# nikhil-lalgudi/distributed-llm-alignment

Hardware: AMD Instinct MI355X
Metric: preference-samples/sec (whole node), Llama-3-8B DPO at 1/2/4/8 MI355X (higher is better)
Workload: dtype bf16; 1 GPU; model=llama3-8b, global_batch=16, seq_len=1024, parallelism=dp1, micro_batch_pairs=4, grad_accum=4, ref_model=frozen, co-resident, backend=single-process, gemm_selection=tunableop:off

## Files before the change

distributed_llm_alignment_amd/csrc/attention.hip:

```cpp
#include <cstdlib>
#include <stdexcept>
#include <type_traits>
#include "common.h"

#include <cstring>
#include "attn_params.h"

namespace dla {

typedef __attribute__((address_space(3))) s16x4 lds_s16x4;

template <int D>
constexpr int attn_dp() { return (D + 31) / 32 * 32; }

template <int W>
__device__ __forceinline__ int swz(int row, int ch) {
  constexpr int NCH = W / 8;
  constexpr int MASK = (NCH & (NCH - 1)) == 0 ? NCH - 1 : 3;
  const int f = (((row & 3) << 2) | ((row >> 2) & 3)) & MASK;
  return row * W + ((ch ^ f) << 3);
}

__device__ __forceinline__ int ds_swz(int row) { return (row >> 1) & 7; }
__device__ __forceinline__ int ds_off(int row, int c4) { return row * 32 + ((c4 ^ ds_swz(row)) << 2); }
// ... 872 lines not shown
      const int t = static_cast<int>(row % T);
      const int64_t bh = row / T;
      const int hh = static_cast<int>(bh % H), b = static_cast<int>(bh / H);
      a[k] = load_bf16x8(o + b * o_sb + t * o_st + hh * o_sh + c);
      g[k] = load_bf16x8(dout + b * do_sb + t * do_st + hh * do_sh + c);
    }
  }
#pragma unroll
  for (int k = 0; k < kDeltaRows; ++k) {
    float acc = 0.f;
#pragma unroll
    for (int j = 0; j < 8; ++j) acc += bf2f(a[k][j]) * bf2f(g[k][j]);
    for (int off = 1; off < lpr; off <<= 1) acc += __shfl_xor(acc, off, 64);
    if (row0 + k < nrows && (lane % lpr) == 0) delta[row0 + k] = acc;
  }
}

template <bool CAUSAL>
__device__ __forceinline__ void bwd_q_range(int k0, int Tq, int causal_off, int window, int& qt0,
                                            int& qend) {
  int qlo = 0, qhi = Tq;
  if (CAUSAL) {
    qlo = max(0, k0 - causal_off);
    if (window > 0) qhi = min(qhi, k0 + kAttnBwdKeys - 1 - causal_off + window);
  }
  qt0 = (qlo / kAttnBwdQRows) * kAttnBwdQRows;
  qend = max(qhi, qt0);
}

template <int D, bool CAUSAL>
// ... 1114 lines not shown
    case 128: fwd_dispatch<128>(p, causal, st); break;
    default: throw std::invalid_argument("attn_fwd: head_dim must be 64, 80 or 128");
  }
}

void launch_attn_bwd_delta(const bf16_t* o, const bf16_t* dout, int64_t o_sb, int64_t o_st,
                           int64_t o_sh, int64_t do_sb, int64_t do_st, int64_t do_sh, int B,
                           int H, int T, int D, float* delta, hipStream_t st) {
  const int64_t rows = static_cast<int64_t>(B) * H * T;
  if (rows == 0) return;
  const int64_t rows_per_block = 4 * (64 / (D <= 64 ? 8 : 16));
  const unsigned nb = static_cast<unsigned>((rows + rows_per_block - 1) / rows_per_block);
  attn_bwd_delta_kernel<<<nb, 256, 0, st>>>(o, dout, o_sb, o_st, o_sh, do_sb, do_st, do_sh, B, H, T, D, delta);
}

static int attn_bwd_waves() {
  const char* e = std::getenv("DLA_ATTN_BWD_WAVES");
  return (e && std::atoi(e) == 4) ? 4 : 8;
}

bool attn_dq_slab_bf16() {
  const char* e = std::getenv("DLA_ATTN_DQ_BF16");
  return attn_bwd_waves() == 8 && !(e && std::atoi(e) == 0);
}

bool attn_dkv_part_bf16() {
  const char* e = std::getenv("DLA_ATTN_DKV_BF16");
  return attn_bwd_waves() == 8 && !(e && std::atoi(e) == 0);
}

// ... 72 lines not shown
```

distributed_llm_alignment_amd/csrc/bindings.cpp:

```cpp
#include <ATen/ATen.h>
#include <ATen/hip/impl/HIPGuardImplMasqueradingAsCUDA.h>
#include <ATen/hip/impl/HIPStreamMasqueradingAsCUDA.h>
#include <torch/library.h>

#include <hip/hip_runtime_api.h>

#include <algorithm>
#include <cstdint>
#include <cstdlib>
#include <tuple>

#include "attn_params.h"
#include "bind_util.h"

namespace dla {

void launch_norm_fwd(const bf16_t*, const bf16_t*, bf16_t*, const bf16_t*, const bf16_t*, bf16_t*,
                     float*, float*, int, int, float, bool, hipStream_t);
void launch_norm_bwd(const bf16_t*, const bf16_t*, const bf16_t*, const float*, const float*,
                     const bf16_t*, bf16_t*, float*, float*, bf16_t*, bf16_t*, int, int, bool,
                     hipStream_t);
int norm_bwd_grid(int rows);
int norm_wgrad_scratch_rows();
void launch_swiglu_fwd(const bf16_t*, bf16_t*, int64_t, int, hipStream_t);
// ... 49 lines not shown
void launch_attn_fwd(const AttnParams&, int, bool, hipStream_t);
int attn_fwd_set_switch(const char* name, int value);
void launch_attn_bwd_delta(const bf16_t*, const bf16_t*, int64_t, int64_t, int64_t, int64_t,
                           int64_t, int64_t, int, int, int, int, float*, hipStream_t);
void launch_attn_bwd(const AttnBwdParams&, int, bool, hipStream_t);
bool attn_dkv_part_bf16();
bool attn_dq_slab_bf16();
void launch_attn_dq_reduce(const float*, int, int, int, int, int, int, bool, int, int,
                           const int*, const int*, int, bf16_t*, int64_t, int64_t, int64_t,
                           const float*, const float*, const int*, int, hipStream_t, const bf16_t*);
void launch_attn_dkv_reduce(const float*, const float*, int, int, int, int, int, float, bf16_t*,
                            int64_t, int64_t, int64_t, bf16_t*, int64_t, int64_t, int64_t,
                            const float*, const float*, const int*, int, hipStream_t, const bf16_t*,
                            const bf16_t*);
void launch_transpose_bf16(const bf16_t*, int64_t, int64_t, int64_t, bf16_t*, int64_t, hipStream_t);

std::tuple<at::Tensor, at::Tensor, at::Tensor, at::Tensor> norm_fwd(
    const at::Tensor& x, const c10::optional<at::Tensor>& res, const at::Tensor& w,
    const c10::optional<at::Tensor>& b, double eps, bool rms) {
  check_bf16(x, "x");
  check_bf16(w, "w");
  TORCH_CHECK(x.is_contiguous(), "x must be contiguous");
  const int64_t H = x.size(-1);
  TORCH_CHECK(H % 8 == 0 && H <= 8192, "norm_fwd: hidden size must be a multiple of 8 and <= 8192");
  TORCH_CHECK(w.numel() == H && w.is_contiguous(), "w shape");
  const int64_t rows = x.numel() / H;
  TORCH_CHECK(rows < (1ll << 31), "too many rows");
  c10::hip::HIPGuardMasqueradingAsCUDA g(x.device());
  auto y = at::empty_like(x);
  at::Tensor so;
// ... 351 lines not shown

static int attn_bwd_hsplit(int64_t nkb, int64_t Hkv, int64_t B, int64_t group, bool causal, int cus) {
  const int64_t base = nkb * Hkv * B;
  const int64_t target = causal ? 2 * static_cast<int64_t>(cus) : cus;
  int hs = 1;
  while (base * hs < target && group % (2 * hs) == 0) hs *= 2;
  return hs;
}

void attn_bwd(const at::Tensor& dout, const at::Tensor& q, const at::Tensor& k,
              const at::Tensor& v, const at::Tensor& o, const at::Tensor& lse2, at::Tensor& dq,
              at::Tensor& dk, at::Tensor& dv, double scale, bool causal, int64_t causal_off,
              int64_t window, const c10::optional<at::Tensor>& kv_start,
              const c10::optional<at::Tensor>& kv_end, const c10::optional<at::Tensor>& segs,
              const c10::optional<at::Tensor>& rope_cos, const c10::optional<at::Tensor>& rope_sin,
              const c10::optional<at::Tensor>& rope_pos, bool rope_inputs) {
  check_bthd(dout, "dout");
  check_bthd(q, "q");
  check_bthd(k, "k");
  check_bthd(v, "v");
  check_bthd(o, "o");
  check_bthd(dq, "dq");
  check_bthd(dk, "dk");
  check_bthd(dv, "dv");
  check_f32(lse2, "lse2");
  const int64_t B = q.size(0), Tq = q.size(1), Hq = q.size(2), D = q.size(3);
  const int64_t Tk = k.size(1), Hkv = k.size(2);
  TORCH_CHECK(D == 64 || D == 80 || D == 128, "head_dim must be 64, 80 or 128");
  TORCH_CHECK(dout.sizes() == q.sizes() && o.sizes() == q.sizes() && dq.sizes() == q.sizes(),
              "dout/o/dq shape");
  TORCH_CHECK(dk.sizes() == k.sizes() && dv.sizes() == v.sizes(), "dk/dv shape");
  TORCH_CHECK(lse2.is_contiguous() && lse2.numel() == B * Hq * Tq, "lse2 shape");
  TORCH_CHECK(Hkv > 0 && Hq % Hkv == 0, "GQA ratio");
  check_kv_range(kv_start, B, "kv_start");
  check_kv_range(kv_end, B, "kv_end");
  c10::hip::HIPGuardMasqueradingAsCUDA g(q.device());
  auto st = cur_stream(q);
  auto fopt = q.options().dtype(at::kFloat);
  auto delta = at::empty({B, Hq, Tq}, fopt);
  launch_attn_bwd_delta(cbp(o), cbp(dout), o.stride(0), o.stride(1), o.stride(2),
                        dout.stride(0), dout.stride(1), dout.stride(2), B, Hq, Tq, D,
                        delta.data_ptr<float>(), st);
  const int64_t nkb = (Tk + kAttnBwdKeys - 1) / kAttnBwdKeys;
  const int64_t slab_rows = (Tq + kAttnBwdQRows - 1) / kAttnBwdQRows * kAttnBwdQRows;
  const bool slab16 = attn_dq_slab_bf16();
  auto slab = at::empty({std::max<int64_t>(nkb, 1), B, slab_rows, Hq, D}, slab16 ? q.options() : fopt);
  const int hs = attn_bwd_hsplit(nkb, Hkv, B, Hq / Hkv, causal, device_cus(q.get_device()));
  at::Tensor dkp, dvp;
  const bool part16 = hs > 1 && attn_dkv_part_bf16();
  if (hs > 1) {
    dkp = at::empty({hs, B, Tk, Hkv, D}, part16 ? q.options() : fopt);
    dvp = at::empty({hs, B, Tk, Hkv, D}, part16 ? q.options() : fopt);
  }
  AttnBwdParams p{};
  p.q = cbp(q); p.k = cbp(k); p.v = cbp(v); p.dout = cbp(dout);
  p.lse2 = lse2.data_ptr<float>(); p.delta = delta.data_ptr<float>();
  p.dq_slab = slab16 ? nullptr : slab.data_ptr<float>();
// ... 27 lines not shown
  launch_attn_bwd(p, static_cast<int>(D), causal, st);
  launch_attn_dq_reduce(p.dq_slab, static_cast<int>(nkb), static_cast<int>(B), static_cast<int>(Tq),
                        p.slab_rows, static_cast<int>(Hq), static_cast<int>(D), causal, p.causal_off, p.window,
                        p.kv_start, p.kv_end, static_cast<int>(Tk), bp(dq), dq.stride(0),
                        dq.stride(1), dq.stride(2), p.rope_cos, p.rope_sin, p.rope_pos, p.rope_rot, st,
                        p.dq_slab16);
  if (hs > 1) {
    launch_attn_dkv_reduce(p.dk_part, p.dv_part, hs, static_cast<int>(B), static_cast<int>(Tk),
                           static_cast<int>(Hkv), static_cast<int>(D), p.scale, bp(dk),
                           dk.stride(0), dk.stride(1), dk.stride(2), bp(dv), dv.stride(0),
                           dv.stride(1), dv.stride(2), p.rope_cos, p.rope_sin, p.rope_pos, p.rope_rot, st,
                           p.dk_part16, p.dv_part16);
  }
}

void transpose_bf16(const at::Tensor& in, at::Tensor& out) {
  check_bf16(in, "in");
  check_bf16(out, "out");
  TORCH_CHECK(in.dim() == 2 && out.dim() == 2 && in.stride(1) == 1 && out.stride(1) == 1 &&
                  out.size(0) == in.size(1) && out.size(1) == in.size(0),
              "transpose_bf16: in [R, C], out [C, R], unit column stride");
  TORCH_CHECK(in.stride(0) % 8 == 0 && out.stride(0) % 8 == 0, "16-byte aligned rows");
  check_aligned16(in, "in");
  check_aligned16(out, "out");
  same_device(in, out);
  c10::hip::HIPGuardMasqueradingAsCUDA g(in.device());
  launch_transpose_bf16(cbp(in), in.size(0), in.size(1), in.stride(0), bp(out), out.stride(0),
                        cur_stream(in));
}

// ... 434 lines not shown

}

TORCH_LIBRARY(dla, m) {
  m.def("norm_fwd(Tensor x, Tensor? res, Tensor w, Tensor? b, float eps, bool rms) -> (Tensor, Tensor, Tensor, Tensor)");
  m.def("norm_bwd(Tensor dy, Tensor s, Tensor w, Tensor rstd, Tensor? mean, Tensor? dres, bool has_bias, bool rms) -> (Tensor, Tensor, Tensor)");
  m.def("swiglu_fwd(Tensor gu) -> Tensor");
  m.def("swiglu_bwd(Tensor gu, Tensor dout) -> Tensor");
  m.def("swiglu_fwd_t(Tensor gu) -> (Tensor, Tensor)");
  m.def("swiglu_bwd_t(Tensor gu, Tensor dout) -> (Tensor, Tensor)");
  m.def("gelu_fwd(Tensor x) -> Tensor");
  m.def("gelu_bwd(Tensor x, Tensor dy) -> Tensor");
  m.def("rope_fwd(Tensor qkv, Tensor cos, Tensor sin, Tensor? pos, int Hq, int Hkv, int D, int rot, int T, int pos_offset) -> (Tensor, Tensor)");
  m.def("rope_bwd(Tensor dq, Tensor dk, Tensor(a!) dqkv, Tensor cos, Tensor sin, Tensor? pos, int Hq, int Hkv, int D, int rot, int T, int pos_offset) -> ()");
  m.def("attn_fwd(Tensor q, Tensor k, Tensor v, float scale, bool causal, int causal_off, int window, Tensor? kv_start, Tensor? kv_end, Tensor? segs=None, Tensor? rope_cos=None, Tensor? rope_sin=None, Tensor? rope_pos=None, Tensor(a!)? q_rot=None, bool rope_k=True) -> (Tensor, Tensor)");
  m.def("attn_bwd(Tensor dout, Tensor q, Tensor k, Tensor v, Tensor o, Tensor lse2, Tensor(a!) dq, Tensor(b!) dk, Tensor(c!) dv, float scale, bool causal, int causal_off, int window, Tensor? kv_start, Tensor? kv_end, Tensor? segs=None, Tensor? rope_cos=None, Tensor? rope_sin=None, Tensor? rope_pos=None, bool rope_inputs=False) -> ()");
  m.def("attn_stamps(Tensor like) -> Tensor");
  m.def("attn_fwd_switch(str name, int value) -> int", &dla::attn_fwd_switch);
  m.def("transpose_bf16(Tensor input, Tensor(a!) out) -> ()");
  m.def("logprob_fwd(Tensor logits, Tensor targets, int vocab_offset=0) -> (Tensor, Tensor)");
  m.def("logprob_bwd(Tensor(a!) logits, Tensor targets, Tensor lse, Tensor grad, int vocab_offset=0) -> ()");
  m.def("logprob_bwd_t(Tensor(a!) logits, Tensor targets, Tensor lse, Tensor grad, int vocab_offset=0) -> Tensor");
  m.def("logprob_entropy_fwd(Tensor logits, Tensor targets, int vocab_offset=0) -> (Tensor, Tensor, Tensor)");
  m.def("logprob_entropy_bwd(Tensor(a!) logits, Tensor targets, Tensor lse, Tensor ent, Tensor grad_logp, Tensor grad_ent, int vocab_offset=0) -> ()");
  m.def("logprob_entropy_bwd_t(Tensor(a!) logits, Tensor targets, Tensor lse, Tensor ent, Tensor grad_logp, Tensor grad_ent, int vocab_offset=0) -> Tensor");
  m.def("row_lse(Tensor logits) -> Tensor");
  m.def("ensemble_kl(Tensor(a!) s_logits, Tensor t_logits, Tensor s_lse, Tensor t_lse, Tensor? grad, bool write_grad) -> Tensor");
  m.def("seq_reduce(Tensor lp, Tensor mask) -> (Tensor, Tensor)");
  m.def("seq_expand_grad(Tensor coef, Tensor mask, Tensor cnt, bool mean) -> Tensor");
  m.def("dpo_loss(Tensor pol, Tensor ref, float beta, float label_smoothing) -> (Tensor, Tensor, Tensor, Tensor)");
  m.def("pairwise_loss(Tensor sc, Tensor sr) -> (Tensor, Tensor, Tensor, Tensor)");
// ... 9 lines not shown
}

TORCH_LIBRARY_IMPL(dla, CUDA, m) {
  m.impl("norm_fwd", &dla::norm_fwd);
  m.impl("norm_bwd", &dla::norm_bwd);
  m.impl("swiglu_fwd", &dla::swiglu_fwd);
  m.impl("swiglu_bwd", &dla::swiglu_bwd);
  m.impl("swiglu_fwd_t", &dla::swiglu_fwd_t);
  m.impl("swiglu_bwd_t", &dla::swiglu_bwd_t);
  m.impl("gelu_fwd", &dla::gelu_fwd);
  m.impl("gelu_bwd", &dla::gelu_bwd);
  m.impl("rope_fwd", &dla::rope_fwd);
  m.impl("rope_bwd", &dla::rope_bwd);
  m.impl("attn_fwd", &dla::attn_fwd);
  m.impl("attn_bwd", &dla::attn_bwd);
  m.impl("attn_stamps", &dla::attn_stamps);
  m.impl("transpose_bf16", &dla::transpose_bf16);
  m.impl("logprob_fwd", &dla::logprob_fwd);
  m.impl("logprob_bwd", &dla::logprob_bwd);
  m.impl("logprob_bwd_t", &dla::logprob_bwd_t);
  m.impl("logprob_entropy_fwd", &dla::logprob_entropy_fwd);
  m.impl("logprob_entropy_bwd", &dla::logprob_entropy_bwd);
  m.impl("logprob_entropy_bwd_t", &dla::logprob_entropy_bwd_t);
  m.impl("row_lse", &dla::row_lse);
  m.impl("ensemble_kl", &dla::ensemble_kl);
  m.impl("seq_reduce", &dla::seq_reduce);
  m.impl("seq_expand_grad", &dla::seq_expand_grad);
  m.impl("dpo_loss", &dla::dpo_loss);
  m.impl("pairwise_loss", &dla::pairwise_loss);
  m.impl("kl_penalty_pg", &dla::kl_penalty_pg);
// ... 10 lines not shown
```

distributed_llm_alignment_amd/csrc/common.h:

```cpp
#pragma once

#include <hip/hip_runtime.h>
#include <stdint.h>

namespace dla {

using bf16_t = uint16_t;

typedef uint16_t bf16x8 __attribute__((ext_vector_type(8)));
typedef uint16_t bf16x4 __attribute__((ext_vector_type(4)));
typedef float f32x4 __attribute__((ext_vector_type(4)));
typedef float f32x16 __attribute__((ext_vector_type(16)));
typedef short s16x8 __attribute__((ext_vector_type(8)));
typedef short s16x4 __attribute__((ext_vector_type(4)));

constexpr int kWave = 64;

__device__ __forceinline__ float bf2f(bf16_t v) {
  return __uint_as_float(static_cast<uint32_t>(v) << 16);
}

typedef float f32x2 __attribute__((ext_vector_type(2)));
typedef __bf16 hbf16x2 __attribute__((ext_vector_type(2)));

// ... 58 lines not shown
  if (l == 0) scratch[w] = v;
  __syncthreads();
  float r = -INFINITY;
#pragma unroll
  for (int i = 0; i < NT / 64; ++i) r = fmaxf(r, scratch[i]);
  return r;
}

__device__ __forceinline__ bf16x8 load_bf16x8(const bf16_t* p) {
  return *reinterpret_cast<const bf16x8*>(p);
}
__device__ __forceinline__ void store_bf16x8(bf16_t* p, bf16x8 v) {
  *reinterpret_cast<bf16x8*>(p) = v;
}

__device__ __forceinline__ float fast_exp(float x) { return __expf(x); }
__device__ __forceinline__ float sigmoidf_(float x) { return 1.f / (1.f + __expf(-x)); }
__device__ __forceinline__ float log_sigmoid(float x) {
  return fminf(x, 0.f) - log1pf(__expf(-fabsf(x)));
}

__device__ __forceinline__ int xcd_remap(int bid, int nblocks) {
  const int q = nblocks / 8, r = nblocks % 8;
  const int xcd = bid % 8, idx = bid / 8;
  return (xcd < r ? xcd * (q + 1) : r * (q + 1) + (xcd - r) * q) + idx;
}

__device__ __forceinline__ s16x8 f8x8_to_bf16(uint32_t w0, uint32_t w1) {
  typedef short s16x2v __attribute__((ext_vector_type(2)));
  const s16x2v a = __builtin_bit_cast(s16x2v, __builtin_amdgcn_cvt_scalef32_pk_bf16_fp8(w0, 1.0f, false));
// ... 9 lines not shown
```

distributed_llm_alignment_amd/models/transformer.py:

```python
from __future__ import annotations

import math
import os
from typing import Dict, List, Optional, Tuple

import torch
import torch.nn as nn
import torch.nn.functional as F
from torch.utils.checkpoint import checkpoint

from .. import ops
from .config import ModelConfig


def _param(*shape, device=None, dtype=None) -> nn.Parameter:
    return nn.Parameter(torch.empty(*shape, device=device, dtype=dtype))


def attention_layout(attention_mask: Optional[torch.Tensor]):
    if attention_mask is None:
        return None, None, None
    m = attention_mask.to(torch.int32)
    first = (m.cumsum(1) == 0).sum(1).to(torch.int32)
    end = first + m.sum(1).to(torch.int32)
    T = m.shape[1]
    pos = (torch.arange(T, device=m.device, dtype=torch.int32).unsqueeze(0) - first.unsqueeze(1)).clamp(min=0)
# ... 19 lines not shown
    def __init__(self, cfg: ModelConfig, device=None, dtype=None):
        super().__init__()
        self.cfg = cfg
        H = cfg.hidden_size
        self.qkv_proj = _param(cfg.q_size + 2 * cfg.kv_size, H, device=device, dtype=dtype)
        self.qkv_bias = _param(cfg.q_size + 2 * cfg.kv_size, device=device, dtype=dtype) if cfg.attn_bias else None
        self.o_proj = _param(H, cfg.q_size, device=device, dtype=dtype)
        o_bias = cfg.attn_bias and cfg.arch in ("gpt2", "phi")
        self.o_bias = _param(H, device=device, dtype=dtype) if o_bias else None
        self.tp = None
        self.tp_seq = None
        self.sp = None
        self.h_local, self.kv_local = cfg.num_heads, cfg.num_kv_heads

    def forward(self, h, rope, kv_start, kv_end, positions, cache=None, layer_idx=0, segs=None,
                resid=None):
        cfg = self.cfg
        seq = self.tp_seq if (h.dim() == 2 and cache is None) else None
        from ..parallel import tensor_parallel as tpm

        sp_overlap = seq is not None and tpm.TP_OVERLAP and self.qkv_bias is None
        if sp_overlap:
            B, T = positions.shape
            qkv = tpm.sp_gather_linear(h, self.qkv_proj, seq).view(B, T, -1)
        elif seq is not None:
            B, T = positions.shape
            h = tpm.sp_gather(h, seq).view(B, T, -1)
        if sp_overlap:
            pass
        elif seq is None and self.tp is not None and torch.is_grad_enabled():
            from ..parallel.tensor_parallel import col_parallel_linear

            qkv = col_parallel_linear(h, self.qkv_proj, self.qkv_bias, self.tp)
        else:
            qkv = _lin(h, self.qkv_proj, self.qkv_bias)
        window = cfg.sliding_window if cfg.sliding_window else 0
        if cache is None and self.sp is not None:
            a = self.sp.attention(
                qkv, self.h_local, self.kv_local, cfg.head_dim,
                lambda full, hq, hkv: ops.qkv_attention(full, hq, hkv, cfg.head_dim, rope, causal=True,
                                                        window=window, kv_start=kv_start, kv_end=kv_end,
                                                        positions=positions, segs=segs))
        elif cache is None:
            a = ops.qkv_attention(qkv, self.h_local, self.kv_local, cfg.head_dim, rope,
                                  causal=True, window=window, kv_start=kv_start, kv_end=kv_end,
                                  positions=positions, segs=segs)
        else:
            a = cache.attend(layer_idx, qkv, rope, window)
        if self.tp is None:
            if resid is not None:
                assert self.o_bias is None
                return ops.linear_add(a, self.o_proj, resid)
            return _lin(a, self.o_proj, self.o_bias)
        assert resid is None
        from ..parallel.tensor_parallel import sp_reduce_scatter, tp_grad_sum, tp_reduce

        if seq is not None:
            if tpm.TP_OVERLAP:
                out = tpm.sp_linear_reduce_scatter(a.reshape(-1, a.shape[-1]), self.o_proj, seq)
            else:
                out = sp_reduce_scatter(ops.linear(a, self.o_proj, None).reshape(-1, cfg.hidden_size), seq)
            return out + tp_grad_sum(self.o_bias, seq) if self.o_bias is not None else out
        from ..parallel.tensor_parallel import row_parallel_linear

        out = row_parallel_linear(a, self.o_proj, self.tp)
        return out + self.o_bias if self.o_bias is not None else out

# ... 122 lines not shown
class DecoderLayer(nn.Module):
    def __init__(self, cfg: ModelConfig, device=None, dtype=None):
        super().__init__()
        self.cfg = cfg
        H = cfg.hidden_size
        bias = cfg.norm_type == "layer"
        self.ln1_w = _param(H, device=device, dtype=dtype)
        self.ln1_b = _param(H, device=device, dtype=dtype) if bias else None
        if not cfg.parallel_block:
            self.ln2_w = _param(H, device=device, dtype=dtype)
            self.ln2_b = _param(H, device=device, dtype=dtype) if bias else None
        self.attn = Attention(cfg, device, dtype)
        self.mlp = MoE(cfg, device, dtype) if cfg.is_moe else MLP(cfg, device, dtype)
        self.tp_seq = None
        self.recompute = None

    def decode_fused_ok(self, x) -> bool:
        cfg, at, mlp = self.cfg, self.attn, self.mlp
        return (cfg.norm_type == "rms" and not cfg.parallel_block and isinstance(mlp, MLP)
                and cfg.activation == "swiglu" and mlp.up_bias is None and mlp.down_bias is None
                and at.qkv_bias is None and at.o_bias is None and at.tp is None and mlp.tp is None
                and at.sp is None and self.ln1_b is None and self.ln2_b is None
                and ops.decode.fused_layer_ok(x, cfg.hidden_size, at.qkv_proj, at.o_proj,
                                              mlp.up_proj, mlp.down_proj))

    def decode_fused(self, s, ssq, rope, cache, layer_idx):
        cfg, at, mlp = self.cfg, self.attn, self.mlp
        if ssq is None:
            h, _ = ops.add_norm(s, None, self.ln1_w, None, cfg.norm_eps, True)
            qkv = _lin(h, at.qkv_proj, None)
# ... 10 lines not shown
        at, mlp = self.attn, self.mlp
        return (FUSED_RESIDUAL and cache is None and seq is None and not self.cfg.parallel_block
                and isinstance(mlp, MLP) and at.tp is None and mlp.tp is None and at.o_bias is None
                and mlp.down_bias is None)

    def forward(self, x, resid, rope, kv_start, kv_end, positions, cache=None, layer_idx=0, segs=None):
        cfg = self.cfg
        rms = cfg.norm_type == "rms"
        seq = self.tp_seq if x.dim() == 2 else None
        if seq is not None:
            from ..parallel.tensor_parallel import tp_grad_sum as w_
        else:
            w_ = _ident
        rc = self.recompute if (cache is None and self.training and torch.is_grad_enabled()) else None
        if self.fused_residual_ok(x, cache, seq):
            h, s = ops.add_norm(x, resid, self.ln1_w, self.ln1_b, cfg.norm_eps, rms, keep_stream=True)
            if rc == "attention":
                s = checkpoint(self.attn, h, rope, kv_start, kv_end, positions, None, layer_idx, segs, s,
                               use_reentrant=False)
            else:
                s = self.attn(h, rope, kv_start, kv_end, positions, None, layer_idx, segs, resid=s)
            h, s = ops.add_norm(s, None, self.ln2_w, self.ln2_b, cfg.norm_eps, rms, keep_stream=True)
            if rc == "mlp":
                return checkpoint(self.mlp, h, s, use_reentrant=False), None
            return self.mlp(h, s), None
        h, resid = ops.add_norm(x, resid, w_(self.ln1_w, seq), w_(self.ln1_b, seq), cfg.norm_eps, rms)
        if rc == "attention":
            a = checkpoint(self.attn, h, rope, kv_start, kv_end, positions, None, layer_idx, segs,
                           use_reentrant=False)
        else:
            a = self.attn(h, rope, kv_start, kv_end, positions, cache, layer_idx, segs)
        mlp = (lambda t: checkpoint(self.mlp, t, use_reentrant=False)) if rc == "mlp" else self.mlp
        if cfg.parallel_block:
            return a + mlp(h), resid
        h, resid = ops.add_norm(a, resid, w_(self.ln2_w, seq), w_(self.ln2_b, seq), cfg.norm_eps, rms)
        return mlp(h), resid
# ... 46 lines not shown
            p.copy_(init_param_tensor(self.cfg, name, idx, tuple(p.shape), seed, p.device, p.dtype))
        return self

    RECOMPUTE_POLICIES = ("full", "mlp", "attention")

    def gradient_checkpointing_enable(self, policy="full", gradient_checkpointing_kwargs=None):
        if policy is True or policy is None:
            policy = "full"
        policy = str(policy).lower()
        if policy not in self.RECOMPUTE_POLICIES:
            raise ValueError(f"gradient checkpointing policy must be one of {self.RECOMPUTE_POLICIES}, "
                             f"got {policy!r}")
        self.gradient_checkpointing = policy == "full"
        for layer in self.layers:
            layer.recompute = None if policy == "full" else policy
        self.recompute_policy = policy

    def gradient_checkpointing_disable(self):
        self.gradient_checkpointing = False
        for layer in self.layers:
            layer.recompute = None
        self.recompute_policy = None

    @property
    def head_weight(self) -> torch.Tensor:
        return self.embed if self.lm_head is None else self.lm_head

    def embed_tokens(self, input_ids, positions=None):
        if self.vocab_parallel is not None:
            from ..parallel.tensor_parallel import vocab_parallel_embedding

            x = vocab_parallel_embedding(input_ids, self.embed, self.vocab_parallel[0], self.tp)
        else:
            x = ops.embedding(input_ids, self.embed)
        if self.wpe is not None:
            T = input_ids.shape[1]
# ... 269 lines not shown
```

distributed_llm_alignment_amd/ops/attention.py:

```python
from __future__ import annotations

import math
import os
from typing import Dict, Optional

import torch
import torch.nn.functional as F

from . import _ext


class RotaryCache:

    def __init__(self, rot_dim: int, theta: float = 10000.0, max_pos: int = 4096,
                 scaling: Optional[dict] = None):
        self.rot_dim = rot_dim
        self.theta = theta
        self.max_pos = max_pos
        inv = 1.0 / (theta ** (torch.arange(0, rot_dim, 2, dtype=torch.float64) / rot_dim))
        if scaling and scaling.get("rope_type", scaling.get("type")) == "llama3":
            factor = scaling.get("factor", 8.0)
            lo = scaling.get("low_freq_factor", 1.0)
            hi = scaling.get("high_freq_factor", 4.0)
            old = scaling.get("original_max_position_embeddings", 8192)
# ... 132 lines not shown
        elif rot == 0:
            q4 = qkv.as_strided((B, T, Hq, D), (T * C, C, D, 1), off)
            k4 = qkv.as_strided((B, T, Hkv, D), (T * C, C, D, 1), off + Hq * D)
        v4 = qkv.as_strided((B, T, Hkv, D), (T * C, C, D, 1), off + (Hq + Hkv) * D)
        do4 = do.contiguous().view(B, T, Hq, D)
        dqkv = torch.empty((B, T, C), dtype=qkv.dtype, device=qkv.device)
        dv = dqkv.as_strided((B, T, Hkv, D), (T * C, C, D, 1), (Hq + Hkv) * D)
        fused_rope = (rot == D and D in (64, 128) or (D == 80 and rot == 32)) and \
            (FUSED_ROPE_BWD or ctx.on_load)
        if rot > 0 and not fused_rope:
            dq = torch.empty((B, T, Hq, D), dtype=qkv.dtype, device=qkv.device)
            dk = torch.empty((B, T, Hkv, D), dtype=qkv.dtype, device=qkv.device)
        else:
            dq = dqkv.as_strided((B, T, Hq, D), (T * C, C, D, 1), 0)
            dk = dqkv.as_strided((B, T, Hkv, D), (T * C, C, D, 1), Hq * D)
        if fused_rope:
            ops.attn_bwd(do4, q4, k4, v4, o, lse2, dq, dk, dv, float(scale), bool(causal), 0,
                         int(window), kv_start, kv_end, segs, cos, sin, pos, bool(ctx.on_load))
        else:
            ops.attn_bwd(do4, q4, k4, v4, o, lse2, dq, dk, dv, float(scale), bool(causal), 0,
                         int(window), kv_start, kv_end, segs)
        if rot > 0 and not fused_rope:
            ops.rope_bwd(dq.view(B * T, Hq * D), dk.view(B * T, Hkv * D), dqkv.view(B * T, C),
                         cos, sin, pos, Hq, Hkv, D, rot, T, 0)
        return dqkv, None, None, None, None, None, None, None, None, None, None, None, None, None


class _AttnCoreFn(torch.autograd.Function):

    @staticmethod
    def forward(ctx, q, k, v, scale, causal, causal_off, window, kv_start, kv_end, segs=None):
        ops = _ext.require()
        o, lse2 = ops.attn_fwd(q, k, v, float(scale), bool(causal), int(causal_off), int(window),
                               kv_start, kv_end, segs)
        ctx.save_for_backward(q, k, v, o, lse2, kv_start, kv_end, segs)
        ctx.cfg = (scale, causal, causal_off, window)
# ... 131 lines not shown
```

distributed_llm_alignment_amd/ops/linear.py:

```python
from __future__ import annotations

import os

import torch
import torch.nn.functional as F

from . import _ext

TRANSPOSED_DGRAD = os.environ.get("DLA_TRANSPOSED_DGRAD", "1") != "0"


def transposed_weight(weight: torch.Tensor) -> torch.Tensor:
    wt = getattr(weight, "_dla_wt", None)
    ep = getattr(weight, "_dla_epoch", None)
    key = (weight._version, ep[0] if ep is not None else 0)
    if wt is None or getattr(weight, "_dla_wt_ver", None) != key:
        with torch.no_grad():
            if wt is None:
                wt = torch.empty((weight.shape[1], weight.shape[0]), dtype=weight.dtype, device=weight.device)
            _ext.require().transpose_bf16(weight.detach(), wt)
        weight._dla_wt = wt
        weight._dla_wt_ver = key
    return wt

# ... 55 lines not shown
    mg = getattr(weight, "main_grad", None)
    if mg is None or getattr(weight, "_dla_shared", False):
        return False
    _wgrad_accumulate(mg, dy2, x2, dyt, xt)
    hook = getattr(weight, "_dla_grad_hook", None)
    if hook is not None:
        hook(weight)
    return True


def uses_main_grad(weight: torch.Tensor) -> bool:
    return (weight.requires_grad and torch.is_grad_enabled() and getattr(weight, "main_grad", None) is not None
            and not getattr(weight, "_dla_shared", False))


class _LinearMainGradFn(torch.autograd.Function):
    @staticmethod
    def forward(ctx, x, weight, bias):
        ctx.save_for_backward(x)
        ctx.weight = weight
        ctx.has_bias = bias is not None
        return F.linear(x, weight, bias)

    @staticmethod
    def backward(ctx, dy):
        (x,) = ctx.saved_tensors
        weight = ctx.weight
        K, N = x.shape[-1], dy.shape[-1]
        dy2 = dy.reshape(-1, N)
        dx = input_grad(dy2, weight).view(x.shape) if ctx.needs_input_grad[0] else None
# ... 65 lines not shown

def add_gemm(x2: torch.Tensor, weight: torch.Tensor, c2: torch.Tensor) -> torch.Tensor:
    if (x2.is_cuda and x2.dtype == torch.bfloat16 and weight.dtype == torch.bfloat16 and c2.dtype == torch.bfloat16
            and x2.stride(-1) == 1 and weight.stride(-1) == 1 and c2.stride(-1) == 1):
        from ..utils.tuning import hipblaslt_solution

        sol = hipblaslt_solution(weight.shape[0], x2.shape[0], x2.shape[1], weight.stride(0), x2.stride(0),
                                 weight.shape[0])
        return _ext.require().linear_add_lt(x2, weight, c2, sol)
    return torch.addmm(c2, x2, weight.t())


class _LinearAddFn(torch.autograd.Function):

    @staticmethod
    def forward(ctx, x, weight, resid):
        ctx.save_for_backward(x)
        ctx.weight = weight
        N = weight.shape[0]
        y = add_gemm(x.reshape(-1, x.shape[-1]), weight, resid.reshape(-1, N))
        return y.view(resid.shape)

    @staticmethod
    def backward(ctx, dy):
        (x,) = ctx.saved_tensors
        weight = ctx.weight
        K, N = x.shape[-1], dy.shape[-1]
        dy2 = dy.reshape(-1, N)
        dx = input_grad(dy2, weight).view(x.shape) if ctx.needs_input_grad[0] else None
        dw = None
        if ctx.needs_input_grad[1]:
            x2 = x.reshape(-1, K)
            if not accumulate_weight_grad(weight, dy2, x2):
                dw = dy2.t() @ x2
        return dx, dw, (dy if ctx.needs_input_grad[2] else None)


def linear_add(x: torch.Tensor, weight: torch.Tensor, resid: torch.Tensor) -> torch.Tensor:
    if fp8_inference_ok(x, weight, None):
        return fp8_linear_frozen(x, weight).add_(resid)
    if torch.is_grad_enabled() and (x.requires_grad or weight.requires_grad or resid.requires_grad):
        return _LinearAddFn.apply(x, weight, resid)
    N = weight.shape[0]
    return add_gemm(x.reshape(-1, x.shape[-1]), weight, resid.reshape(-1, N)).view(resid.shape)


def linear(x: torch.Tensor, weight: torch.Tensor, bias=None) -> torch.Tensor:
    if fp8_inference_ok(x, weight, bias):
        return fp8_linear_frozen(x, weight)
    if uses_main_grad(weight):
        return _LinearMainGradFn.apply(x, weight, bias)
    return F.linear(x, weight, bias)
```

distributed_llm_alignment_amd/parallel/data_parallel.py:

```python
from __future__ import annotations

import contextlib
import os
from dataclasses import dataclass, field
from typing import Dict, List, Optional

import torch
import torch.distributed as dist
import torch.nn as nn

from ..optim.adamw import adamw_update, clip_coefficient, grad_sumsq
from .dist import DistState, ExposedCommTimer, state as dist_state
from . import collectives as coll

ALIGN = 64


@dataclass
class Bucket:
    start: int
    end: int
    params: List[nn.Parameter] = field(default_factory=list)
    shard_off: int = 0
    expert: bool = False
    group: object = None
# ... 316 lines not shown
                self._sumsq = dense + self._esumsq
            else:
                ew = self.buckets[[b.expert for b in self.buckets].index(True)].world
                self._sumsq = dense / self.world + self._esumsq / ew
            coll.all_reduce(self._sumsq, op=dist.ReduceOp.SUM, group=self.group)
        elif self.zero and self._comm:
            coll.all_reduce(self._sumsq, op=dist.ReduceOp.SUM, group=self.group)
        if self.tp_size > 1:
            coll.all_reduce(self._sumsq, op=dist.ReduceOp.SUM, group=self.tp_group)
        sumsq = self._sumsq * (gs * gs)
        norm, coef = clip_coefficient(sumsq, self.max_grad_norm if self.max_grad_norm else 0.0)
        self.last_grad_norm = norm
        return coef

    def step(self, lr: Optional[float] = None) -> torch.Tensor:
        self.finish_grad_sync()
        self.comm_timer.close_step()
        lr = self.lr if lr is None else lr
        coef = self.clip_and_norm()
        self.step_count += 1
        adamw_update(self.param_shard, self.master, self.grad_shard, self.exp_avg, self.exp_avg_sq,
                     lr, self.betas[0], self.betas[1], self.eps, self.wd, self.step_count,
                     clip=coef if self.max_grad_norm else None, grad_scale=self.grad_scale)
        if self.zero:
            self.wait_params()
            for bi in reversed(range(len(self.buckets))):
                b = self.buckets[bi]
                c = b.size // b.world
                if b.world == 1 and not self.force_comm:
                    if not self.shard_alias:
# ... 109 lines not shown
```

distributed_llm_alignment_amd/parallel/fsdp.py:

```python
from __future__ import annotations

import contextlib
import os
from typing import Dict, List, Optional

import torch
import torch.distributed as dist
import torch.nn as nn

from ..optim.adamw import adamw_update, clip_coefficient, grad_sumsq
from .dist import DistState, ExposedCommTimer, state as dist_state
from . import collectives as coll

ALIGN = 64


def _round_up(x: int, m: int) -> int:
    return (x + m - 1) // m * m


def _free(t: torch.Tensor) -> None:
    st = t.untyped_storage()
    if st.size() != 0:
        st.resize_(0)
# ... 410 lines not shown
    def clip_and_norm(self):
        gs = self.grad_scale
        grad_sumsq(self.grad_shard, self._sumsq, accumulate=False)
        if self._repl_ranges:
            rep = sum(self.grad_shard[a:e].float().pow(2).sum() for a, e in self._repl_ranges)
            self._sumsq -= (1.0 - 1.0 / self.tp_size) * rep
        if self._comm:
            coll.all_reduce(self._sumsq, op=dist.ReduceOp.SUM, group=self.group)
        if self.tp_size > 1:
            coll.all_reduce(self._sumsq, op=dist.ReduceOp.SUM, group=self.tp_group)
        norm, coef = clip_coefficient(self._sumsq * (gs * gs), self.max_grad_norm or 0.0)
        self.last_grad_norm = norm
        return coef

    def step(self, lr: Optional[float] = None) -> torch.Tensor:
        self.finish_grad_sync()
        self.comm_timer.close_step()
        lr = self.lr if lr is None else lr
        coef = self.clip_and_norm()
        self.step_count += 1
        self._wt_epoch[0] += 1
        adamw_update(self.param_shard, self.master, self.grad_shard, self.exp_avg, self.exp_avg_sq,
                     lr, self.betas[0], self.betas[1], self.eps, self.wd, self.step_count,
                     clip=coef if self.max_grad_norm else None, grad_scale=self.grad_scale)
        root = self.units[-1]
        root.resident = False
        self._gather(root)
        self.zero_grad()
        return self.last_grad_norm

# ... 101 lines not shown
```

Measured before the change: 10.20 preference_pairs/s.

## Fuse attention delta computation with o_proj input transpose in backward

In the o_proj backward, a new kernel reads the attention output and its gradient once. From those reads it computes the row-wise delta (dot of O and dO) and also writes a transposed copy of O for the weight-gradient GEMM. The delta is passed to the attention backward through a small keyed handoff cache, so attn_bwd skips its own delta kernel. The aim is to remove a separate pass over O/dO and a separate transpose. In exchange it adds global state keyed on tensor pointer and version, which could go stale or mismatch.

```diff
diff --git a/distributed_llm_alignment_amd/csrc/attention.hip b/distributed_llm_alignment_amd/csrc/attention.hip
--- a/distributed_llm_alignment_amd/csrc/attention.hip
+++ b/distributed_llm_alignment_amd/csrc/attention.hip
@@ -910,6 +910,56 @@
     for (int off = 1; off < lpr; off <<= 1) acc += __shfl_xor(acc, off, 64);
     if (row0 + k < nrows && (lane % lpr) == 0) delta[row0 + k] = acc;
   }
+}
+
+template <int D>
+__global__ __launch_bounds__(256) void attn_bwd_delta_t_kernel(const bf16_t* __restrict__ o,
+                                                                const bf16_t* __restrict__ dout,
+                                                                int B, int H, int T,
+                                                                float* __restrict__ delta,
+                                                                bf16_t* __restrict__ oT) {
+  constexpr int NP = D / 64;
+  const int lane = threadIdx.x & 63, c = lane & 7;
+  const int h = blockIdx.y * 4 + (threadIdx.x >> 6);
+  const int64_t ntok = static_cast<int64_t>(B) * T;
+  const int64_t tok0 = static_cast<int64_t>(blockIdx.x) * 64 + (lane >> 3) * 8;
+  if (h >= H || tok0 >= ntok) return;
+  const int64_t HD = static_cast<int64_t>(H) * D;
+  bf16x8 a[NP][8];
+  float acc[NP][8];
+#pragma unroll
+  for (int p = 0; p < NP; ++p) {
+    bf16x8 g[8];
+#pragma unroll
+    for (int i = 0; i < 8; ++i) {
+      const int64_t off = (tok0 + i) * HD + static_cast<int64_t>(h) * D + p * 64 + c * 8;
+      a[p][i] = load_bf16x8(o + off);
+      g[i] = load_bf16x8(dout + off);
+    }
+#pragma unroll
+    for (int i = 0; i < 8; ++i) {
+      float s = 0.f;
+#pragma unroll
+      for (int j = 0; j < 8; ++j) s += bf2f(a[p][i][j]) * bf2f(g[i][j]);
+      acc[p][i] = s;
+    }
+  }
+  float d[8];
+#pragma unroll
+  for (int i = 0; i < 8; ++i) {
+#pragma unroll
+    for (int p = 0; p < NP; ++p)
+      for (int off = 1; off < 8; off <<= 1) acc[p][i] += __shfl_xor(acc[p][i], off, 64);
+    d[i] = NP == 2 ? acc[0][i] + acc[NP - 1][i] : acc[0][i];
+  }
+  if (c == 0) {
+    const int b = static_cast<int>(tok0 / T), t0 = static_cast<int>(tok0 % T);
+    float* dp = delta + (static_cast<int64_t>(b) * H + h) * T + t0;
+    *reinterpret_cast<f32x4*>(dp) = f32x4{d[0], d[1], d[2], d[3]};
+    *reinterpret_cast<f32x4*>(dp + 4) = f32x4{d[4], d[5], d[6], d[7]};
+  }
+#pragma unroll
+  for (int p = 0; p < NP; ++p) store_block_t(a[p], oT, ntok, static_cast<int64_t>(h) * D + p * 64 + c * 8, tok0);
 }
 
 template <bool CAUSAL>
@@ -2054,6 +2104,15 @@
   attn_bwd_delta_kernel<<<nb, 256, 0, st>>>(o, dout, o_sb, o_st, o_sh, do_sb, do_st, do_sh, B, H, T, D, delta);
 }
 
+bool launch_attn_bwd_delta_t(const bf16_t* o, const bf16_t* dout, int B, int H, int T, int D,
+                             float* delta, bf16_t* oT, hipStream_t st) {
+  if ((D != 64 && D != 128) || T <= 0 || T % 8 != 0 || B <= 0 || H <= 0) return false;
+  const dim3 grid(static_cast<unsigned>((static_cast<int64_t>(B) * T + 63) / 64), (H + 3) / 4);
+  if (D == 64) attn_bwd_delta_t_kernel<64><<<grid, 256, 0, st>>>(o, dout, B, H, T, delta, oT);
+  else attn_bwd_delta_t_kernel<128><<<grid, 256, 0, st>>>(o, dout, B, H, T, delta, oT);
+  return true;
+}
+
 static int attn_bwd_waves() {
   const char* e = std::getenv("DLA_ATTN_BWD_WAVES");
   return (e && std::atoi(e) == 4) ? 4 : 8;
diff --git a/distributed_llm_alignment_amd/csrc/bindings.cpp b/distributed_llm_alignment_amd/csrc/bindings.cpp
--- a/distributed_llm_alignment_amd/csrc/bindings.cpp
+++ b/distributed_llm_alignment_amd/csrc/bindings.cpp
@@ -87,6 +87,7 @@
                             const float*, const float*, const int*, int, hipStream_t, const bf16_t*,
                             const bf16_t*);
 void launch_transpose_bf16(const bf16_t*, int64_t, int64_t, int64_t, bf16_t*, int64_t, hipStream_t);
+bool launch_attn_bwd_delta_t(const bf16_t*, const bf16_t*, int, int, int, int, float*, bf16_t*, hipStream_t);
 
 std::tuple<at::Tensor, at::Tensor, at::Tensor, at::Tensor> norm_fwd(
     const at::Tensor& x, const c10::optional<at::Tensor>& res, const at::Tensor& w,
@@ -468,7 +469,8 @@
               int64_t window, const c10::optional<at::Tensor>& kv_start,
               const c10::optional<at::Tensor>& kv_end, const c10::optional<at::Tensor>& segs,
               const c10::optional<at::Tensor>& rope_cos, const c10::optional<at::Tensor>& rope_sin,
-              const c10::optional<at::Tensor>& rope_pos, bool rope_inputs) {
+              const c10::optional<at::Tensor>& rope_pos, bool rope_inputs,
+              const c10::optional<at::Tensor>& delta_in) {
   check_bthd(dout, "dout");
   check_bthd(q, "q");
   check_bthd(k, "k");
@@ -491,10 +493,18 @@
   c10::hip::HIPGuardMasqueradingAsCUDA g(q.device());
   auto st = cur_stream(q);
   auto fopt = q.options().dtype(at::kFloat);
-  auto delta = at::empty({B, Hq, Tq}, fopt);
-  launch_attn_bwd_delta(cbp(o), cbp(dout), o.stride(0), o.stride(1), o.stride(2),
-                        dout.stride(0), dout.stride(1), dout.stride(2), B, Hq, Tq, D,
-                        delta.data_ptr<float>(), st);
+  at::Tensor delta;
+  if (delta_in && delta_in->defined()) {
+    check_f32(*delta_in, "delta");
+    TORCH_CHECK(delta_in->is_contiguous() && delta_in->numel() == B * Hq * Tq, "delta shape");
+    same_device(q, *delta_in);
+    delta = *delta_in;
+  } else {
+    delta = at::empty({B, Hq, Tq}, fopt);
+    launch_attn_bwd_delta(cbp(o), cbp(dout), o.stride(0), o.stride(1), o.stride(2),
+                          dout.stride(0), dout.stride(1), dout.stride(2), B, Hq, Tq, D,
+                          delta.data_ptr<float>(), st);
+  }
   const int64_t nkb = (Tk + kAttnBwdKeys - 1) / kAttnBwdKeys;
   const int64_t slab_rows = (Tq + kAttnBwdQRows - 1) / kAttnBwdQRows * kAttnBwdQRows;
   const bool slab16 = attn_dq_slab_bf16();
@@ -552,6 +562,27 @@
   }
 }
 
+std::tuple<at::Tensor, at::Tensor> attn_delta_t(const at::Tensor& o, const at::Tensor& dout) {
+  check_bthd(o, "o");
+  check_bthd(dout, "dout");
+  TORCH_CHECK(o.sizes() == dout.sizes(), "o/dout shape");
+  same_device(o, dout);
+  const int64_t B = o.size(0), T = o.size(1), H = o.size(2), D = o.size(3);
+  auto fopt = o.options().dtype(at::kFloat);
+  if (!o.is_contiguous() || !dout.is_contiguous() || (D != 64 && D != 128) || T % 8 != 0 || B * T * H == 0)
+    return {at::empty({0}, fopt), at::empty({0}, o.options())};
+  check_aligned16(o, "o");
+  check_aligned16(dout, "dout");
+  c10::hip::HIPGuardMasqueradingAsCUDA g(o.device());
+  auto delta = at::empty({B, H, T}, fopt);
+  auto oT = at::empty({H * D, B * T}, o.options());
+  const bool ok = launch_attn_bwd_delta_t(cbp(o), cbp(dout), static_cast<int>(B), static_cast<int>(H),
+                                          static_cast<int>(T), static_cast<int>(D), delta.data_ptr<float>(),
+                                          bp(oT), cur_stream(o));
+  TORCH_CHECK(ok, "attn_delta_t: launcher refused a shape the binding accepted");
+  return {delta, oT};
+}
+
 void transpose_bf16(const at::Tensor& in, at::Tensor& out) {
   check_bf16(in, "in");
   check_bf16(out, "out");
@@ -1016,7 +1047,8 @@
   m.def("rope_fwd(Tensor qkv, Tensor cos, Tensor sin, Tensor? pos, int Hq, int Hkv, int D, int rot, int T, int pos_offset) -> (Tensor, Tensor)");
   m.def("rope_bwd(Tensor dq, Tensor dk, Tensor(a!) dqkv, Tensor cos, Tensor sin, Tensor? pos, int Hq, int Hkv, int D, int rot, int T, int pos_offset) -> ()");
   m.def("attn_fwd(Tensor q, Tensor k, Tensor v, float scale, bool causal, int causal_off, int window, Tensor? kv_start, Tensor? kv_end, Tensor? segs=None, Tensor? rope_cos=None, Tensor? rope_sin=None, Tensor? rope_pos=None, Tensor(a!)? q_rot=None, bool rope_k=True) -> (Tensor, Tensor)");
-  m.def("attn_bwd(Tensor dout, Tensor q, Tensor k, Tensor v, Tensor o, Tensor lse2, Tensor(a!) dq, Tensor(b!) dk, Tensor(c!) dv, float scale, bool causal, int causal_off, int window, Tensor? kv_start, Tensor? kv_end, Tensor? segs=None, Tensor? rope_cos=None, Tensor? rope_sin=None, Tensor? rope_pos=None, bool rope_inputs=False) -> ()");
+  m.def("attn_bwd(Tensor dout, Tensor q, Tensor k, Tensor v, Tensor o, Tensor lse2, Tensor(a!) dq, Tensor(b!) dk, Tensor(c!) dv, float scale, bool causal, int causal_off, int window, Tensor? kv_start, Tensor? kv_end, Tensor? segs=None, Tensor? rope_cos=None, Tensor? rope_sin=None, Tensor? rope_pos=None, bool rope_inputs=False, Tensor? delta=None) -> ()");
+  m.def("attn_delta_t(Tensor o, Tensor dout) -> (Tensor, Tensor)");
   m.def("attn_stamps(Tensor like) -> Tensor");
   m.def("attn_fwd_switch(str name, int value) -> int", &dla::attn_fwd_switch);
   m.def("transpose_bf16(Tensor input, Tensor(a!) out) -> ()");
@@ -1056,6 +1088,7 @@
   m.impl("rope_bwd", &dla::rope_bwd);
   m.impl("attn_fwd", &dla::attn_fwd);
   m.impl("attn_bwd", &dla::attn_bwd);
+  m.impl("attn_delta_t", &dla::attn_delta_t);
   m.impl("attn_stamps", &dla::attn_stamps);
   m.impl("transpose_bf16", &dla::transpose_bf16);
   m.impl("logprob_fwd", &dla::logprob_fwd);
diff --git a/distributed_llm_alignment_amd/csrc/common.h b/distributed_llm_alignment_amd/csrc/common.h
--- a/distributed_llm_alignment_amd/csrc/common.h
+++ b/distributed_llm_alignment_amd/csrc/common.h
@@ -96,6 +96,14 @@
   *reinterpret_cast<bf16x8*>(p) = v;
 }
 
+__device__ __forceinline__ void store_block_t(const bf16x8 (&rows)[8], bf16_t* dstT, int64_t ldT,
+                                              int64_t col0, int64_t row0) {
+  bf16x8 tt[8];
+  tr8_bf16(rows, tt);
+#pragma unroll
+  for (int j = 0; j < 8; ++j) store_bf16x8(dstT + (col0 + j) * ldT + row0, tt[j]);
+}
+
 __device__ __forceinline__ float fast_exp(float x) { return __expf(x); }
 __device__ __forceinline__ float sigmoidf_(float x) { return 1.f / (1.f + __expf(-x)); }
 __device__ __forceinline__ float log_sigmoid(float x) {
diff --git a/distributed_llm_alignment_amd/models/transformer.py b/distributed_llm_alignment_amd/models/transformer.py
--- a/distributed_llm_alignment_amd/models/transformer.py
+++ b/distributed_llm_alignment_amd/models/transformer.py
@@ -10,6 +10,8 @@
 from torch.utils.checkpoint import checkpoint
 
 from .. import ops
+from ..ops import _handoff
+from ..ops.attention import NATIVE_HEAD_DIMS
 from .config import ModelConfig
 
 
@@ -59,7 +61,7 @@
         self.h_local, self.kv_local = cfg.num_heads, cfg.num_kv_heads
 
     def forward(self, h, rope, kv_start, kv_end, positions, cache=None, layer_idx=0, segs=None,
-                resid=None):
+                resid=None, producer_t=False):
         cfg = self.cfg
         seq = self.tp_seq if (h.dim() == 2 and cache is None) else None
         from ..parallel import tensor_parallel as tpm
@@ -80,6 +82,8 @@
         else:
             qkv = _lin(h, self.qkv_proj, self.qkv_bias)
         window = cfg.sliding_window if cfg.sliding_window else 0
+        fused_core = (producer_t and cache is None and self.sp is None and self.tp is None and h.dim() == 3
+                      and cfg.head_dim in NATIVE_HEAD_DIMS and ops._ext.use_native(h))
         if cache is None and self.sp is not None:
             a = self.sp.attention(
                 qkv, self.h_local, self.kv_local, cfg.head_dim,
@@ -95,7 +99,8 @@
         if self.tp is None:
             if resid is not None:
                 assert self.o_bias is None
-                return ops.linear_add(a, self.o_proj, resid)
+                return ops.linear_add(a, self.o_proj, resid,
+                                      attn_heads=(self.h_local, cfg.head_dim) if fused_core else None)
             return _lin(a, self.o_proj, self.o_bias)
         assert resid is None
         from ..parallel.tensor_parallel import sp_reduce_scatter, tp_grad_sum, tp_reduce
@@ -248,6 +253,7 @@
         self.mlp = MoE(cfg, device, dtype) if cfg.is_moe else MLP(cfg, device, dtype)
         self.tp_seq = None
         self.recompute = None
+        self.recompute_full = False
 
     def decode_fused_ok(self, x) -> bool:
         cfg, at, mlp = self.cfg, self.attn, self.mlp
@@ -288,12 +294,14 @@
             w_ = _ident
         rc = self.recompute if (cache is None and self.training and torch.is_grad_enabled()) else None
         if self.fused_residual_ok(x, cache, seq):
+            pt = (_handoff.PRODUCER_T and rc != "attention" and not self.recompute_full and torch.is_grad_enabled())
             h, s = ops.add_norm(x, resid, self.ln1_w, self.ln1_b, cfg.norm_eps, rms, keep_stream=True)
             if rc == "attention":
                 s = checkpoint(self.attn, h, rope, kv_start, kv_end, positions, None, layer_idx, segs, s,
                                use_reentrant=False)
             else:
-                s = self.attn(h, rope, kv_start, kv_end, positions, None, layer_idx, segs, resid=s)
+                s = self.attn(h, rope, kv_start, kv_end, positions, None, layer_idx, segs, resid=s,
+                              producer_t=pt)
             h, s = ops.add_norm(s, None, self.ln2_w, self.ln2_b, cfg.norm_eps, rms, keep_stream=True)
             if rc == "mlp":
                 return checkpoint(self.mlp, h, s, use_reentrant=False), None
@@ -370,12 +378,14 @@
         self.gradient_checkpointing = policy == "full"
         for layer in self.layers:
             layer.recompute = None if policy == "full" else policy
+            layer.recompute_full = policy == "full"
         self.recompute_policy = policy
 
     def gradient_checkpointing_disable(self):
         self.gradient_checkpointing = False
         for layer in self.layers:
             layer.recompute = None
+            layer.recompute_full = False
         self.recompute_policy = None
 
     @property
diff --git a/distributed_llm_alignment_amd/ops/_handoff.py b/distributed_llm_alignment_amd/ops/_handoff.py
--- /dev/null
+++ b/distributed_llm_alignment_amd/ops/_handoff.py
@@ -0,0 +1,43 @@
+from __future__ import annotations
+
+import os
+from collections import deque
+from typing import Any, Dict, Optional
+
+import torch
+
+PRODUCER_T = os.environ.get("DLA_PRODUCER_T", "1") != "0"
+
+MAX_ENTRIES = 4
+
+_entries: deque = deque()
+
+
+def _key(t: torch.Tensor):
+    return (t.data_ptr(), tuple(t.shape), tuple(t.stride()), t.dtype, t.device, t._version)
+
+
+def offer(grad: torch.Tensor, **extras: Any) -> None:
+    _entries.append((_key(grad), grad, extras))
+    while len(_entries) > MAX_ENTRIES:
+        _entries.popleft()
+
+
+def take(grad: Optional[torch.Tensor]) -> Dict[str, Any]:
+    if grad is None or not _entries:
+        return {}
+    key = _key(grad)
+    for i in range(len(_entries) - 1, -1, -1):
+        if _entries[i][0] == key:
+            extras = _entries[i][2]
+            del _entries[i]
+            return extras
+    return {}
+
+
+def clear() -> None:
+    _entries.clear()
+
+
+def pending() -> int:
+    return len(_entries)
diff --git a/distributed_llm_alignment_amd/ops/attention.py b/distributed_llm_alignment_amd/ops/attention.py
--- a/distributed_llm_alignment_amd/ops/attention.py
+++ b/distributed_llm_alignment_amd/ops/attention.py
@@ -7,7 +7,7 @@
 import torch
 import torch.nn.functional as F
 
-from . import _ext
+from . import _ext, _handoff
 
 
 class RotaryCache:
@@ -170,12 +170,13 @@
         else:
             dq = dqkv.as_strided((B, T, Hq, D), (T * C, C, D, 1), 0)
             dk = dqkv.as_strided((B, T, Hkv, D), (T * C, C, D, 1), Hq * D)
+        delta = _handoff.take(do).get("delta")
         if fused_rope:
             ops.attn_bwd(do4, q4, k4, v4, o, lse2, dq, dk, dv, float(scale), bool(causal), 0,
-                         int(window), kv_start, kv_end, segs, cos, sin, pos, bool(ctx.on_load))
+                         int(window), kv_start, kv_end, segs, cos, sin, pos, bool(ctx.on_load), delta)
         else:
             ops.attn_bwd(do4, q4, k4, v4, o, lse2, dq, dk, dv, float(scale), bool(causal), 0,
-                         int(window), kv_start, kv_end, segs)
+                         int(window), kv_start, kv_end, segs, None, None, None, False, delta)
         if rot > 0 and not fused_rope:
             ops.rope_bwd(dq.view(B * T, Hq * D), dk.view(B * T, Hkv * D), dqkv.view(B * T, C),
                          cos, sin, pos, Hq, Hkv, D, rot, T, 0)
diff --git a/distributed_llm_alignment_amd/ops/linear.py b/distributed_llm_alignment_amd/ops/linear.py
--- a/distributed_llm_alignment_amd/ops/linear.py
+++ b/distributed_llm_alignment_amd/ops/linear.py
@@ -5,7 +5,7 @@
 import torch
 import torch.nn.functional as F
 
-from . import _ext
+from . import _ext, _handoff
 
 TRANSPOSED_DGRAD = os.environ.get("DLA_TRANSPOSED_DGRAD", "1") != "0"
 
@@ -93,6 +93,12 @@
             and not getattr(weight, "_dla_shared", False))
 
 
+def wgrad_takes_t(weight: torch.Tensor, M: int) -> bool:
+    mg = getattr(weight, "main_grad", None)
+    return (_handoff.PRODUCER_T and weight.requires_grad and mg is not None
+            and not getattr(weight, "_dla_shared", False) and _tn_ok(mg, M))
+
+
 class _LinearMainGradFn(torch.autograd.Function):
     @staticmethod
     def forward(ctx, x, weight, bias):
@@ -188,9 +194,10 @@
 class _LinearAddFn(torch.autograd.Function):
 
     @staticmethod
-    def forward(ctx, x, weight, resid):
+    def forward(ctx, x, weight, resid, attn_heads=None):
         ctx.save_for_backward(x)
         ctx.weight = weight
+        ctx.attn_heads = attn_heads
         N = weight.shape[0]
         y = add_gemm(x.reshape(-1, x.shape[-1]), weight, resid.reshape(-1, N))
         return y.view(resid.shape)
@@ -205,16 +212,26 @@
         dw = None
         if ctx.needs_input_grad[1]:
             x2 = x.reshape(-1, K)
-            if not accumulate_weight_grad(weight, dy2, x2):
+            M = x2.shape[0]
+            xt = None
+            if (ctx.attn_heads is not None and dx is not None and x.dim() == 3 and x.is_contiguous()
+                    and wgrad_takes_t(weight, M)):
+                Hq, D = ctx.attn_heads
+                B, T = x.shape[0], x.shape[1]
+                delta, ot = _ext.require().attn_delta_t(x.view(B, T, Hq, D), dx.view(B, T, Hq, D))
+                if ot.numel():
+                    xt = ot
+                    _handoff.offer(dx, delta=delta)
+            if not accumulate_weight_grad(weight, dy2, x2, None, xt):
                 dw = dy2.t() @ x2
-        return dx, dw, (dy if ctx.needs_input_grad[2] else None)
-
-
-def linear_add(x: torch.Tensor, weight: torch.Tensor, resid: torch.Tensor) -> torch.Tensor:
+        return dx, dw, (dy if ctx.needs_input_grad[2] else None), None
+
+
+def linear_add(x: torch.Tensor, weight: torch.Tensor, resid: torch.Tensor, attn_heads=None) -> torch.Tensor:
     if fp8_inference_ok(x, weight, None):
         return fp8_linear_frozen(x, weight).add_(resid)
     if torch.is_grad_enabled() and (x.requires_grad or weight.requires_grad or resid.requires_grad):
-        return _LinearAddFn.apply(x, weight, resid)
+        return _LinearAddFn.apply(x, weight, resid, attn_heads if _handoff.PRODUCER_T else None)
     N = weight.shape[0]
     return add_gemm(x.reshape(-1, x.shape[-1]), weight, resid.reshape(-1, N)).view(resid.shape)
 
diff --git a/distributed_llm_alignment_amd/parallel/data_parallel.py b/distributed_llm_alignment_amd/parallel/data_parallel.py
--- a/distributed_llm_alignment_amd/parallel/data_parallel.py
+++ b/distributed_llm_alignment_amd/parallel/data_parallel.py
@@ -9,6 +9,7 @@
 import torch.distributed as dist
 import torch.nn as nn
 
+from ..ops import _handoff
 from ..optim.adamw import adamw_update, clip_coefficient, grad_sumsq
 from .dist import DistState, ExposedCommTimer, state as dist_state
 from . import collectives as coll
@@ -355,6 +356,7 @@
         return coef
 
     def step(self, lr: Optional[float] = None) -> torch.Tensor:
+        _handoff.clear()
         self.finish_grad_sync()
         self.comm_timer.close_step()
         lr = self.lr if lr is None else lr
diff --git a/distributed_llm_alignment_amd/parallel/fsdp.py b/distributed_llm_alignment_amd/parallel/fsdp.py
--- a/distributed_llm_alignment_amd/parallel/fsdp.py
+++ b/distributed_llm_alignment_amd/parallel/fsdp.py
@@ -8,6 +8,7 @@
 import torch.distributed as dist
 import torch.nn as nn
 
+from ..ops import _handoff
 from ..optim.adamw import adamw_update, clip_coefficient, grad_sumsq
 from .dist import DistState, ExposedCommTimer, state as dist_state
 from . import collectives as coll
@@ -448,6 +449,7 @@
         return coef
 
     def step(self, lr: Optional[float] = None) -> torch.Tensor:
+        _handoff.clear()
         self.finish_grad_sync()
         self.comm_timer.close_step()
         lr = self.lr if lr is None else lr
```

Measured after the change: 10.26 preference_pairs/s, median of 6. Within noise of the previous version (+0.5%).
